# lukifer23/Matrix0

Hardware: AMD Instinct MI355X
Metric: self-play games/sec at 800 sims/move, ResNet-24 53M; 1/2/4/8 MI355X (higher is better)
Workload: dtype f16

## Files before the change

### matrix0_amd/csrc/capi_selfplay.hip

```cpp
#include <string.h>
#include <algorithm>
#include <memory>
#include "selfplay_engine.h"

using namespace m0;

static void fill_tree_cfg(const m0_selfplay_cfg& c, bool match, TreeCfg& t) {
    t.fpu_reduction = c.fpu_reduction; t.draw_penalty = c.draw_penalty; t.virtual_loss = c.virtual_loss;
    t.selection_jitter = c.selection_jitter; t.cpuct = c.cpuct; t.cpuct_start = c.cpuct_start; t.cpuct_end = c.cpuct_end;
    t.cpuct_plies = c.cpuct_plies; t.use_c_base = c.use_c_base; t.cpuct_c_base = c.cpuct_c_base; t.cpuct_c_init = c.cpuct_c_init;
    t.dirichlet_alpha = c.dirichlet_alpha; t.dirichlet_frac = c.dirichlet_frac; t.legal_softmax = c.legal_softmax;
    t.enable_entropy_noise = c.enable_entropy_noise; t.no_instant_backtrack = c.no_instant_backtrack;
    t.virtual_loss_active = c.virtual_loss_active; t.leaves_per_step = c.inference_batch_size;
    t.tt_merge = c.tt_merge; t.raw_legal_priors = c.raw_legal_priors; t.max_children = c.max_children;
    t.min_child_prior = c.min_child_prior;
    t.eval_cache = ((match ? c.arena_eval_cache : c.eval_cache) && c.legal_softmax && !c.raw_legal_priors && !c.tt_merge) ? 1 : 0;
}

static void alloc_tree_arenas(m0_selfplay* sp) {
    const m0_selfplay_cfg& c = sp->cfg;
    long want = c.arena_nodes > 0 ? c.arena_nodes : (long)(c.num_simulations * 1.3 + 64) * 96;
    if (want < 4096) want = 4096;
    sp->cap = (int)want;
    const size_t N = (size_t)sp->G * 2 * sp->cap;
    TreeArrays& t = sp->d.t;
    t.cap = sp->cap;
    t.prior = dalloc<double>(sp, N); t.w = dalloc<double>(sp, N); t.q = dalloc<double>(sp, N);
    t.n = dalloc<int>(sp, N); t.vl = dalloc<int>(sp, N); t.cbase = dalloc<int>(sp, N);
    t.nch = dalloc<int16_t>(sp, N); t.mv = dalloc<uint16_t>(sp, N); t.midx = dalloc<uint16_t>(sp, N);
    sp->d.games = dalloc<GameDev>(sp, sp->G);
    const size_t LS = (size_t)sp->L + 1;
    sp->d.samples = dalloc<Sample>(sp, (size_t)sp->G * LS);
    sp->d.paths = dalloc<int>(sp, (size_t)sp->G * LS * M0_MAX_DEPTH);
    sp->d.leaf_moves = dalloc<uint16_t>(sp, (size_t)sp->G * LS * M0_MAX_CHILDREN);
}

static bool alloc_position_tables(m0_selfplay* sp) {
    sp->d.tt_sides = 1;
    if (!sp->cfg.tt_merge) return true;
    const size_t LS = (size_t)sp->L + 1;
    int tc = 1024;
    while (tc < 2 * sp->cap) tc <<= 1;
    sp->d.tt_cap = tc;
    sp->d.tt_sides = sp->kind == EngineKind::Match ? 2 : 1;
    sp->d.search_nodes = (int)std::min<long>((long)sp->cfg.num_simulations * 48 + 4 * M0_MAX_CHILDREN, (long)sp->cap / 2);
    sp->d.epaths = dalloc<int>(sp, (size_t)sp->G * LS * M0_MAX_DEPTH);
    sp->d.tt_keys = dalloc<uint64_t>(sp, (size_t)sp->G * sp->d.tt_sides * tc);
    sp->d.tt_nodes = dalloc<int>(sp, (size_t)sp->G * sp->d.tt_sides * tc);
    if (sp->d.epaths && sp->d.tt_keys && sp->d.tt_nodes) return true;
    m0_set_error("hipMalloc failed for the position tables (tt_merge): lower concurrent_games or arena_nodes");
    return false;
}

static bool alloc_eval_cache(m0_selfplay* sp) {
    if (!sp->tc.eval_cache) return true;
    const size_t LS = (size_t)sp->L + 1;
    int entries = sp->cfg.eval_cache_entries > 0 ? sp->cfg.eval_cache_entries : 16384;
    int sets = 64;
    while (sets * 4 < entries) sets <<= 1;
    EvalCache& ec = sp->d.ec;
    ec.sets = sets;
    ec.sides = sp->kind == EngineKind::Match ? 2 : 1;
    const size_t entries_all = (size_t)sp->G * ec.sides * sets * 4;
    ec.keys = dalloc<uint64_t>(sp, entries_all);
    ec.stamps = dalloc<uint32_t>(sp, entries_all);
    ec.payload = dalloc<float>(sp, entries_all * M0_EC_WORDS);
    ec.hit_stage = dalloc<float>(sp, (size_t)sp->G * LS * M0_EC_WORDS);
    if (ec.keys && ec.stamps && ec.payload && ec.hit_stage) return true;
    m0_set_error("hipMalloc failed for the evaluation cache: lower eval_cache_entries or concurrent_games");
    return false;
}

static bool alloc_batch_buffers(m0_selfplay* sp) {
    const int nreg = sp->kind == EngineKind::Match ? 2 : 1;
    sp->d.hist = dalloc<uint64_t>(sp, (size_t)sp->G * M0_HIST_CAP);
    sp->d.results = dalloc<RootResult>(sp, sp->G);
    sp->d.row_counter = dalloc<int>(sp, 4);
    sp->d.x0 = dalloc<_Float16>(sp, (size_t)(nreg * sp->rows_max + 4) * 64 * 32);
    sp->logits_dev = dalloc<float>(sp, (size_t)nreg * sp->rows_max * 4672);
    sp->values_dev = dalloc<float>(sp, (size_t)nreg * sp->rows_max + 4);
    sp->d.net_row_base = sp->rows_max;
    if (sp->cfg.ssl_in_forward && sp->net && sp->net->ssl_channels_total() > 0)
        sp->ssl_dev = dalloc<float>(sp, (size_t)sp->rows_max * sp->net->ssl_channels_total() * 64);
    if (sp->cfg.ssl_targets) {
        sp->ssl_cap = sp->cfg.max_game_len > 0 ? sp->cfg.max_game_len + 1 : 513;
        sp->ssl_pos_dev = dalloc<Pos>(sp, sp->ssl_cap);
        sp->ssl_out_dev = dalloc<float>(sp, (size_t)sp->ssl_cap * 17 * 64);
        if (!sp->ssl_pos_dev || !sp->ssl_out_dev) {
            m0_set_error("hipMalloc failed for the SSL target staging buffers");
            return false;
        }
    }
    sp->ids_dev = dalloc<int>(sp, sp->G);
    sp->roots_dev = dalloc<int>(sp, sp->G);
    sp->d.logits = sp->logits_dev; sp->d.values = sp->values_dev;
    sp->d.G = sp->G; sp->d.L = sp->L;
    return true;
}

static bool make_tail_view(m0_selfplay* sp) {
    if (!(sp->cfg.tail_split && sp->net && sp->kind != EngineKind::Match && sp->net->cfg().channels > 256 && sp->net->cfg().channels <= 320 &&
          sp->rows_max >= 2048)) return true;
    if (create_stream_cu_mask_env("M0_TAIL_CU_MASK", &sp->stream_tail) != hipSuccess ||
        hipEventCreateWithFlags(&sp->ev_sel, hipEventDisableTiming) != hipSuccess ||
        hipEventCreateWithFlags(&sp->ev_tail, hipEventDisableTiming) != hipSuccess) {
        m0_set_error("hipStreamCreate / hipEventCreate failed (tail split)");
        return false;
    }
    sp->net_tail = sp->net->shared_view(sp->stream_tail);
    std::string werr;
    sp->half_split = sp->cfg.tail_split == 2;
    if (sp->net_tail->ensure_workspace(sp->half_split ? sp->rows_max / 2 + 1024 : 1023, werr) != M0_OK) {
        m0_set_error("tail split: " + werr);
        return false;
    }
    return true;
}
// ... 318 lines not shown
```

### matrix0_amd/csrc/tree.h

```cpp
#pragma once
#include <hip/hip_runtime.h>
#include <stdint.h>
#include "chess_core.h"
namespace m0 { struct TbSet; }
#include "../../include/m0_engine.h"

#define M0_MAX_DEPTH 256
#define M0_HIST_CAP 192
#define M0_MAX_CHILDREN 256
constexpr int M0_NHWC_C = 32;

struct TreeCfg {
    double fpu_reduction;
    double draw_penalty;
    double virtual_loss;
    double selection_jitter;
    double cpuct;
    double cpuct_start, cpuct_end;
    int cpuct_plies;
    int use_c_base;
    double cpuct_c_base, cpuct_c_init;
    double dirichlet_alpha, dirichlet_frac;
    int legal_softmax;
    int enable_entropy_noise;
// ... 17 lines not shown
    int sets;
    int sides;
};

struct GameDev {
    m0::Pos root_pos;
    int root;
    int next;
    int arena;
    int active;
    int sims_done, sims_target;
    int need_dirichlet;
    int root_q_from_v;
    int flip_root_v;
    int root_fresh;
    int hist_len;
    int nsamples;
    int overflow;
    int finished;
    int root_n;
    double root_q;
    double root_v;
    uint64_t seed_jitter, seed_noise, seed_dir;
    uint64_t ctr_jitter, ctr_noise, ctr_dir;
    uint64_t evals;
    int net_id;
    int reinfer;
    uint64_t cache_hits;
    uint32_t cache_clock[2];
    int ec_clear;
    int side_next[2];
    int root_found;
    uint64_t tb_leaves;
};

enum SampleKind : int {
    SK_NONE = 0,
    SK_EVAL = 1,
    SK_ROOT_INIT = 2,
    SK_TERMINAL = 3,
    SK_ROOT_VALUE = 4,
    SK_CACHED = 5,
    SK_SHARED = 6,
};
M0_HD bool sample_owns_row(int kind) { return kind == SK_EVAL || kind == SK_ROOT_INIT || kind == SK_ROOT_VALUE; }
M0_HD bool sample_holds_inflight(int kind) { return kind == SK_EVAL || kind == SK_TERMINAL || kind == SK_CACHED || kind == SK_SHARED; }

struct Sample {
    m0::Pos pos;
    int kind;
    uint64_t ckey;
    int leaf;
    int depth;
    int row;
    int nlegal;
};
static_assert(sizeof(Sample) == 104, "the host copies Sample arrays device-to-host: the layout must not move");

struct TreeArrays {
    double* prior;
    double* w;
    double* q;
    int* n;
    int* vl;
    int* cbase;
    int16_t* nch;
    uint16_t* mv;
    uint16_t* midx;
    int cap;
};

struct RootResult {
    int nchild;
    int root_n;
    double root_q;
    int child_node[M0_MAX_CHILDREN];
    int child_n[M0_MAX_CHILDREN];
    uint16_t child_mv[M0_MAX_CHILDREN];
    uint16_t child_idx[M0_MAX_CHILDREN];
    double child_prior[M0_MAX_CHILDREN];
    double child_q[M0_MAX_CHILDREN];
};

struct TreeDev {
    TreeArrays t;
    GameDev* games;
    Sample* samples;
    int* paths;
    int* epaths;
    uint64_t* tt_keys;
    int* tt_nodes;
    int tt_cap;
    EvalCache ec;
    int search_nodes;
    int tt_sides;
    uint16_t* leaf_moves;
    uint64_t* hist;
    RootResult* results;
    int* row_counter;
    int net_row_base;
    _Float16* x0;
    const float* logits;
    const float* values;
    int G;
    int L;
    const m0::TbSet* tb_set;
    int tb_max_pieces;
};

hipError_t launch_select(const TreeDev& d, const TreeCfg& c, hipStream_t st);
hipError_t launch_expand(const TreeDev& d, const TreeCfg& c, hipStream_t st);
enum RootMode : int {
    ROOT_FRESH = -1,
    ROOT_FROM_SIDE_TABLE = -2,
    ROOT_FIRST_OF_GAME = -3,
};
hipError_t launch_advance(const TreeDev& d, const int* game_ids_dev, const int* child_slots_dev, int count, hipStream_t st);

hipError_t launch_encode_positions(const m0::Pos* pos_dev, int n, float* planes_f32_dev ,
                                   _Float16* nhwc_dev , uint8_t* mask_dev ,
                                   int32_t* nlegal_dev, uint16_t* moves_dev , int32_t* idx_dev ,
                                   hipStream_t st);

hipError_t launch_decode_planes(const float* planes_dev, const uint8_t* mask_dev, int n, m0::Pos* pos_dev, int32_t* status_dev,
                                int32_t* flags_dev, int32_t* nlegal_dev, hipStream_t st);

hipError_t launch_analysis_lines(const TreeDev& d, const int* slots_dev, int count, int multipv, int pv_len,
                                 m0_analysis_line* lines_dev, int* nlines_dev, hipStream_t st);
hipError_t launch_root_children(const TreeDev& d, const int* slots_dev, int count, int32_t* policy_idx_dev, int32_t* visits_dev,
                                int32_t* nchild_dev, hipStream_t st);
hipError_t launch_policy_lines(const float* logits_dev, const float* values_dev, const int32_t* nlegal_dev, const uint16_t* moves_dev,
                               const int32_t* idx_dev, int rows, int multipv, m0_analysis_line* lines_dev, int* nlines_dev,
                               float* value_out_dev, hipStream_t st);

hipError_t launch_ssl_targets(const m0::Pos* pos_dev, int n, float* out_dev, hipStream_t st);

hipError_t launch_replay_games(const m0::Pos* start_dev, const uint32_t* patterns_dev, const int32_t* offsets_dev ,
                               int n_games, int max_plies, m0::Pos* pos_dev, uint16_t* moves_dev, int32_t* policy_idx_dev,
                               int32_t* nlegal_dev, int8_t* turn_dev, int32_t* plies_dev, int32_t* status_dev,
                               int32_t* end_flags_dev, hipStream_t st);
```

### matrix0_amd/csrc/tree_device.h

```cpp
#pragma once
#include <hip/hip_runtime.h>
#include <math.h>
#include "tree.h"

using namespace m0;

#define GOLDEN64 0x9E3779B97F4A7C15ull

__device__ __forceinline__ double u01(uint64_t seed, uint64_t k) {
    return (double)(mix64(seed + (k + 1) * GOLDEN64) >> 11) * (1.0 / 9007199254740992.0);
}
__device__ __forceinline__ double normal_at(uint64_t seed, uint64_t k) {
    double u1 = u01(seed, k), u2 = u01(seed, k + 1);
    if (u1 < 1e-300) u1 = 1e-300;
    return sqrt(-2.0 * log(u1)) * cos(2.0 * 3.141592653589793 * u2);
}
static __device__ double gamma_draw(uint64_t seed, uint64_t& ctr, double a) {
    double boost = 1.0;
    if (a < 1.0) {
        double u = u01(seed, ctr++);
        boost = pow(u, 1.0 / a);
        a += 1.0;
    }
    const double d = a - 1.0 / 3.0, c = 1.0 / sqrt(9.0 * d);
    for (int it = 0; it < 1000; ++it) {
        double x = normal_at(seed, ctr); ctr += 2;
        double v = 1.0 + c * x;
        if (v <= 0.0) continue;
        v = v * v * v;
        double u = u01(seed, ctr++);
        if (u < 1e-300) u = 1e-300;
        if (log(u) < 0.5 * x * x + d - d * v + d * log(v)) return d * v * boost;
    }
    return d * boost;
}

struct Arena {
    double* prior; double* w; double* q; int* n; int* vl; int* cbase; int16_t* nch; uint16_t* mv; uint16_t* midx;
};
__device__ __forceinline__ Arena arena_of(const TreeArrays& t, int g, int half) {
    size_t b = ((size_t)g * 2 + half) * (size_t)t.cap;
    Arena a;
    a.prior = t.prior + b; a.w = t.w + b; a.q = t.q + b; a.n = t.n + b; a.vl = t.vl + b;
    a.cbase = t.cbase + b; a.nch = t.nch + b; a.mv = t.mv + b; a.midx = t.midx + b;
    return a;
}
__device__ __forceinline__ void node_reset(const Arena& A, int i, double prior, Move mv, uint16_t midx) {
    A.prior[i] = prior; A.w[i] = 0.0; A.q[i] = 0.0; A.n[i] = 0; A.vl[i] = 0;
    A.cbase[i] = -1; A.nch[i] = -1; A.mv[i] = mv; A.midx[i] = midx;
}
__device__ __forceinline__ void node_copy(const Arena& D, int dn, const Arena& S, int so) {
    D.prior[dn] = S.prior[so]; D.w[dn] = S.w[so]; D.q[dn] = S.q[so]; D.n[dn] = S.n[so]; D.vl[dn] = 0;
    D.cbase[dn] = S.cbase[so]; D.nch[dn] = S.nch[so]; D.mv[dn] = S.mv[so]; D.midx[dn] = S.midx[so];
}

__device__ __forceinline__ float wave_max_f(float v) {
    for (int o = 32; o > 0; o >>= 1) v = fmaxf(v, __shfl_xor(v, o));
    return v;
}
__device__ __forceinline__ float wave_sum_f(float v) {
    for (int o = 32; o > 0; o >>= 1) v += __shfl_xor(v, o);
    return v;
}
__device__ __forceinline__ double wave_sum_d(double v) {
    for (int o = 32; o > 0; o >>= 1) v += __shfl_xor(v, o);
    return v;
}

constexpr int CPL = M0_MAX_CHILDREN / 64;
static_assert(M0_POLICY_SIZE % 4 == 0, "logit rows are read as 16-byte pieces");

__device__ __forceinline__ bool row_nonfinite(const float* lg, int lane) {
    constexpr int N4 = M0_POLICY_SIZE / 4, PER_LANE = (N4 + 63) / 64;
    const uint4* lg4 = reinterpret_cast<const uint4*>(lg);
    uint4 v[PER_LANE];
#pragma unroll
    for (int k = 0; k < PER_LANE; ++k) { const int j = lane + 64 * k; v[k] = lg4[j < N4 ? j : N4 - 1]; }
    uint32_t acc = 0;
#pragma unroll
    for (int k = 0; k < PER_LANE; ++k) {
        acc |= (uint32_t)((v[k].x & 0x7f800000u) == 0x7f800000u) | (uint32_t)((v[k].y & 0x7f800000u) == 0x7f800000u) |
               (uint32_t)((v[k].z & 0x7f800000u) == 0x7f800000u) | (uint32_t)((v[k].w & 0x7f800000u) == 0x7f800000u);
    }
    return acc != 0;
}

__device__ __forceinline__ void wave_softmax(const float (&l)[CPL], int n, int lane, float (&pr)[CPL]) {
    float mx = -3.0e38f;
#pragma unroll
    for (int k = 0; k < CPL; ++k) mx = fmaxf(mx, l[k]);
    mx = wave_max_f(mx);
    double e[CPL], sum = 0.0;
#pragma unroll
    for (int k = 0; k < CPL; ++k) { const int i = lane + 64 * k; e[k] = i < n ? exp((double)(l[k] - mx)) : 0.0; sum += e[k]; }
    sum = wave_sum_d(sum);
#pragma unroll
    for (int k = 0; k < CPL; ++k) pr[k] = (float)(e[k] / sum);
}

__device__ __forceinline__ int reserve_row(const TreeDev& d, const GameDev* gd, int lane) {
    int row = 0;
    if (lane == 0) row = atomicAdd(d.row_counter + gd->net_id, 1) + gd->net_id * d.net_row_base;
    return __shfl(row, 0);
}
__device__ __forceinline__ double root_value(const GameDev* gd, float v) {
    double rv = fmax(-1.0, fmin(1.0, (double)v));
    if (gd->flip_root_v) rv = -rv;
    return rv;
}

__device__ __forceinline__ uint64_t tt_key_of(const Pos& p) { const uint64_t k = tkey(p); return k ? k : 1ull; }
__device__ __forceinline__ int tt_home(uint64_t key, int cap) { return (int)((key ^ (key >> 29)) & (uint64_t)(cap - 1)); }
__device__ __forceinline__ size_t tt_table_of(const TreeDev& d, int g, const GameDev* gd) {
    return ((size_t)g * d.tt_sides + (d.tt_sides == 2 ? gd->arena : 0)) * (size_t)d.tt_cap;
}
__device__ __forceinline__ void tt_clear(uint64_t* keys, int nkeys, int lane) {
    uint4* tk = reinterpret_cast<uint4*>(keys);
    for (int i = lane; i < nkeys / 2; i += 64) tk[i] = make_uint4(0, 0, 0, 0);
}
static __device__ int tt_lookup(const uint64_t* keys, const int* nodes, int cap, uint64_t key, int lane) {
    const int mask = cap - 1, home = tt_home(key, cap);
    for (int it = 0; it < cap; it += 64) {
        const uint64_t k = keys[(home + it + lane) & mask];
        const unsigned long long hit = __ballot(k == key), emp = __ballot(k == 0ull);
        const int fh = hit ? __builtin_ctzll(hit) : 64, fe = emp ? __builtin_ctzll(emp) : 64;
        if (fh < fe) return nodes[(home + it + fh) & mask];
        if (fe < 64) return -1;
    }
    return -1;
}
static __device__ void tt_insert(uint64_t* keys, int* nodes, int cap, uint64_t key, int node) {
    const int mask = cap - 1;
    int s = tt_home(key, cap);
    for (int it = 0; it < cap; ++it) {
        const unsigned long long prev = atomicCAS(reinterpret_cast<unsigned long long*>(keys + s), 0ull, (unsigned long long)key);
        if (prev == 0ull || prev == (unsigned long long)key) { nodes[s] = node; return; }
        s = (s + 1) & mask;
    }
}

struct NoMirror { __device__ __forceinline__ void operator()(int, int, double) const {} };
template <typename Mirror>
static __device__ void backprop(const Arena& A, const int* path, int depth, double value, int lane, bool may_repeat,
                                const Mirror& mirror) {
    const double v = fmax(-1.0, fmin(1.0, value));
    if (may_repeat) {
        bool dup = false;
        for (int d = lane; d <= depth; d += 64) {
            const int nd = path[d];
// ... 26 lines not shown
```

### matrix0_amd/csrc/tree_expand.hip

```cpp
#include "tree_device.h"
#include "eval_cache.h"

struct ExpandScratch {
    float pr[M0_MAX_CHILDREN];
    uint8_t keep[M0_MAX_CHILDREN];
    float total;
    int bad;
};

struct ExpandEnv {
    Arena A;
    int cap;
    GameDev* gd;
    uint64_t* TK; int* TN; int tt_cap;
    ExpandScratch* X;
    int lane;
};
struct LeafLogits {
    const float* row;
    const float* legal;
    float* store;
};
__device__ __forceinline__ LeafLogits logits_of_row(const float* row, float* store) { return LeafLogits{row, nullptr, store}; }
__device__ __forceinline__ LeafLogits logits_of_cache(const float* payload) { return LeafLogits{nullptr, payload + EC_LOGITS, nullptr}; }

static __device__ float np_sum_f32_dev(const float* a, int n) {
    auto block = [&](const float* b, int m) -> float {
        if (m < 8) { float r = 0.f; for (int i = 0; i < m; ++i) r += b[i]; return r; }
        float r[8];
        for (int j = 0; j < 8; ++j) r[j] = b[j];
        int i;
        for (i = 8; i < m - (m % 8); i += 8)
            for (int j = 0; j < 8; ++j) r[j] += b[i + j];
        float res = ((r[0] + r[1]) + (r[2] + r[3])) + ((r[4] + r[5]) + (r[6] + r[7]));
        for (; i < m; ++i) res += b[i];
        return res;
    };
    if (n <= 128) return block(a, n);
    int n2 = n / 2;
    n2 -= n2 % 8;
    return block(a, n2) + block(a + n2, n - n2);
}

__device__ __forceinline__ void priors_raw(const float* lg, const int (&idx)[CPL], int n, int lane, ExpandScratch* X, float (&pr)[CPL]) {
#pragma unroll
    for (int k = 0; k < CPL; ++k) { const int i = lane + 64 * k; if (i < n) X->pr[i] = lg[idx[k]]; }
    __syncthreads();
    if (lane == 0) X->total = np_sum_f32_dev(X->pr, n);
    __syncthreads();
    const float total = X->total;
    const bool ok = isfinite(total) && total > 0.f;
#pragma unroll
    for (int k = 0; k < CPL; ++k) { const int i = lane + 64 * k; pr[k] = i < n ? (ok ? X->pr[i] / total : 1.0f / (float)n) : 0.f; }
    __syncthreads();
}

__device__ __forceinline__ void priors_uniform(int n, float (&pr)[CPL]) {
#pragma unroll
    for (int k = 0; k < CPL; ++k) pr[k] = 1.0f / (float)n;
}

__device__ __forceinline__ void priors_legal_softmax(const LeafLogits& src, const int (&idx)[CPL], int n, int lane, GameDev* gd,
                                                     const TreeCfg& c, float (&pr)[CPL]) {
    double ent = 0.0;
    float l[CPL];
#pragma unroll
    for (int k = 0; k < CPL; ++k) {
        const int i = lane + 64 * k;
        l[k] = i < n ? (src.legal ? src.legal[i] : src.row[idx[k]]) : -3.0e38f;
        if (src.store && i < n && i < M0_EC_MAXLEGAL) src.store[EC_LOGITS + i] = l[k];
    }
    wave_softmax(l, n, lane, pr);
#pragma unroll
    for (int k = 0; k < CPL; ++k) {
        const int i = lane + 64 * k;
        if (i < n) ent -= (double)pr[k] * log((double)pr[k] + 1e-8);
    }
    ent = wave_sum_d(ent);
    const double ratio = ent / fmax(1e-9, log((double)(n > 1 ? n : 1)));
    if (c.enable_entropy_noise && ratio > 0.9) {
        const uint64_t ctr = gd->ctr_noise;
        const uint64_t seed = gd->seed_noise;
        double dd[CPL], ds = 0.0;
#pragma unroll
        for (int k = 0; k < CPL; ++k) {
            const int i = lane + 64 * k;
            dd[k] = 0.0;
            if (i < n) { dd[k] = fmax((double)pr[k] + 0.1 * normal_at(seed, ctr + 2ull * (uint64_t)i), 1e-8); ds += dd[k]; }
        }
        ds = wave_sum_d(ds);
#pragma unroll
        for (int k = 0; k < CPL; ++k) pr[k] = (float)(dd[k] / ds);
        if (lane == 0) gd->ctr_noise = ctr + 2ull * (uint64_t)n;
    }
}

__device__ __forceinline__ void priors_full_softmax(const float* lg, const int (&idx)[CPL], int n, int lane, GameDev* gd,
                                                    const TreeCfg& c, float (&pr)[CPL]) {
    float mx = -3.0e38f;
    double ent = 0.0;
    for (int j = lane; j < M0_POLICY_SIZE; j += 64) mx = fmaxf(mx, lg[j]);
    mx = wave_max_f(mx);
    double sum = 0.0;
    for (int j = lane; j < M0_POLICY_SIZE; j += 64) sum += exp((double)(lg[j] - mx));
    sum = wave_sum_d(sum);
    const double fsum = sum;
    for (int j = lane; j < M0_POLICY_SIZE; j += 64) {
        const double pj = (double)(float)(exp((double)(lg[j] - mx)) / sum);
        ent -= pj * log(pj + 1e-8);
    }
#pragma unroll
    for (int k = 0; k < CPL; ++k) { const int i = lane + 64 * k; pr[k] = i < n ? (float)(exp((double)(lg[idx[k]] - mx)) / sum) : 0.f; }
    ent = wave_sum_d(ent);
    const double ratio = ent / fmax(1e-9, log((double)(n > 1 ? n : 1)));
    if (c.enable_entropy_noise && ratio > 0.9) {
        const uint64_t ctr = gd->ctr_noise;
        const uint64_t seed = gd->seed_noise;
        double ds = 0.0;
        for (int j = lane; j < M0_POLICY_SIZE; j += 64)
            ds += fmax((double)(float)(exp((double)(lg[j] - mx)) / fsum) + 0.1 * normal_at(seed, ctr + 2ull * (uint64_t)j), 1e-8);
        ds = wave_sum_d(ds);
#pragma unroll
        for (int k = 0; k < CPL; ++k) {
            const int i = lane + 64 * k;
            if (i < n) {
                const int j = idx[k];
                pr[k] = (float)(fmax((double)pr[k] + 0.1 * normal_at(seed, ctr + 2ull * (uint64_t)j), 1e-8) / ds);
            }
        }
        if (lane == 0) gd->ctr_noise = ctr + 2ull * (uint64_t)M0_POLICY_SIZE;
    }
}

__device__ __forceinline__ void priors_renormalise(int n, int lane, float (&pr)[CPL]) {
    double tot = 0.0;
#pragma unroll
    for (int k = 0; k < CPL; ++k) { const int i = lane + 64 * k; if (i < n) { if (!(pr[k] >= 0.f) || !isfinite(pr[k])) pr[k] = 0.f; tot += (double)pr[k]; } }
    tot = wave_sum_d(tot);
    const float totf = (float)tot;
    if (totf > 0.f && isfinite(totf)) {
#pragma unroll
        for (int k = 0; k < CPL; ++k) pr[k] = pr[k] / totf;
    } else priors_uniform(n, pr);
}

__device__ __forceinline__ int prune_children(const TreeCfg& c, const float (&pr)[CPL], int n, int lane, ExpandScratch* X, int (&slot)[CPL]) {
#pragma unroll
    for (int k = 0; k < CPL; ++k) slot[k] = lane + 64 * k;
    if (!(c.max_children > 0 || c.min_child_prior > 0.0)) return n;
#pragma unroll
    for (int k = 0; k < CPL; ++k) {
        const int i = lane + 64 * k;
        if (i < n) { X->pr[i] = pr[k]; X->keep[i] = (c.min_child_prior > 0.0 && !((double)pr[k] >= c.min_child_prior)) ? 0 : 1; }
    }
    __syncthreads();
    int kept = 0;
    for (int j = 0; j < n; ++j) kept += X->keep[j];
    const bool topk = c.max_children > 0 && kept > c.max_children;
    const int nkeep = topk ? c.max_children : kept;
#pragma unroll
    for (int k = 0; k < CPL; ++k) {
        const int i = lane + 64 * k;
        slot[k] = -1;
        if (i < n && X->keep[i]) {
            int r = 0;
            if (topk) { for (int j = 0; j < n; ++j) r += (X->keep[j] && (X->pr[j] > pr[k] || (X->pr[j] == pr[k] && j < i))) ? 1 : 0; }
            else { for (int j = 0; j < i; ++j) r += X->keep[j]; }
            if (r < nkeep) slot[k] = r;
        }
    }
    __syncthreads();
    return nkeep;
}

__device__ __forceinline__ bool write_children(const ExpandEnv& E, int leaf, const Pos& pos, const Move (&mvv)[CPL], const int (&idx)[CPL],
                                               const float (&pr)[CPL], const int (&slot)[CPL], int n, int nkeep, bool reg_children) {
    const Arena& A = E.A;
    GameDev* gd = E.gd;
    const int lane = E.lane;
    const int cb = gd->next;
    if (cb + nkeep > E.cap) { if (lane == 0) gd->overflow = 1; return false; }
#pragma unroll
    for (int k = 0; k < CPL; ++k) {
        const int i = lane + 64 * k;
        if (i < n && slot[k] >= 0) {
            const int ci = cb + slot[k];
            node_reset(A, ci, (double)pr[k], mvv[k], (uint16_t)idx[k]);
            if (E.TK && reg_children) {
                Pos q = pos;
                make_move(q, mvv[k]);
                tt_insert(E.TK, E.TN, E.tt_cap, tt_key_of(q), ci);
            }
        }
    }
    if (E.TK && !reg_children && lane == 0) tt_insert(E.TK, E.TN, E.tt_cap, tt_key_of(pos), leaf);
    if (lane == 0) { A.cbase[leaf] = cb; A.nch[leaf] = (int16_t)nkeep; gd->next = cb + nkeep; }
    __syncthreads();
    return true;
}

__device__ __forceinline__ bool expand_node(const ExpandEnv& E, const TreeCfg& c, int leaf, const Pos& pos, const uint16_t* smoves, int n,
                                   const LeafLogits& src, bool is_root, bool reg_children) {
    const int lane = E.lane;
    if (n <= 0) return true;
    bool bad = false;
    if (!src.legal) bad = row_nonfinite(src.row, lane);
    bad = __any(bad);
    if (lane == 0) E.X->bad = bad ? 1 : 0;
    float pr[CPL];
    int idx[CPL];
    Move mvv[CPL];
#pragma unroll
    for (int k = 0; k < CPL; ++k) {
        const int i = lane + 64 * k;
        pr[k] = 0.f; idx[k] = 0; mvv[k] = 0;
        if (i < n) { mvv[k] = smoves[i]; idx[k] = move_to_index(pos, mvv[k]); }
    }
    if (c.raw_legal_priors && c.legal_softmax && !is_root) priors_raw(src.row, idx, n, lane, E.X, pr);
    else if (bad) priors_uniform(n, pr);
    else {
        if (c.legal_softmax) priors_legal_softmax(src, idx, n, lane, E.gd, c, pr);
        else priors_full_softmax(src.row, idx, n, lane, E.gd, c, pr);
        priors_renormalise(n, lane, pr);
    }
    int slot[CPL];
    const int nkeep = prune_children(c, pr, n, lane, E.X, slot);
    return write_children(E, leaf, pos, mvv, idx, pr, slot, n, nkeep, reg_children);
}

__device__ __forceinline__ void expand_evaluated(const TreeDev& d, const TreeCfg& c, const ExpandEnv& E, int g, const Sample& smp,
                                                 const uint16_t* moves, const float* lg, float v) {
    const Arena& A = E.A;
    GameDev* gd = E.gd;
    const int lane = E.lane, kind = smp.kind, leaf = smp.leaf;
    const Pos pos = smp.pos;
    float* cw = nullptr;
    size_t ce = 0;
    const uint64_t ckey = kind == SK_EVAL ? smp.ckey : 0ull;
    if (ckey != 0 && isfinite(v)) {
        ce = ec_choose_victim(d.ec, gd, g, ckey, lane);
        cw = ec_payload(d.ec, ce);
        ec_invalidate(d.ec, ce, lane);
    }
    const bool ok = expand_node(E, c, leaf, pos, moves, smp.nlegal, logits_of_row(lg, cw), kind == SK_ROOT_INIT,
                                !(kind == SK_ROOT_INIT && gd->root_fresh));
    if (c.eval_cache && kind == SK_EVAL && lane == 0 && A.nch[leaf] < 0) A.cbase[leaf] = -1;
    const int sig = cw ? legal_sig(moves, smp.nlegal, lane) : 0;
    if (cw && lane == 0) {
        if (ok && !E.X->bad) ec_publish(d.ec, gd, ce, ckey, v, sig);
    }
}

__device__ __forceinline__ void release_inflight(const TreeDev& d, const TreeCfg& c, const Arena& A, int g, const Sample* S, const int* P,
                                                 int ns, int lane) {
    for (int s = lane; s < ns; s += 64) {
        if (sample_holds_inflight(S[s].kind)) {
            const int* path = (c.tt_merge ? d.epaths + (size_t)g * (d.L + 1) * M0_MAX_DEPTH : P) + (size_t)s * M0_MAX_DEPTH;
            for (int dd = 1; dd <= S[s].depth; ++dd) atomicSub(&A.vl[path[dd]], 1);
        }
    }
}

__device__ __forceinline__ void write_root_result(RootResult* R, const Arena& A, int root, int lane) {
    const int k = A.nch[root] > 0 ? A.nch[root] : 0;
    const int cb = A.cbase[root];
    for (int i = lane; i < k; i += 64) {
        R->child_node[i] = cb + i; R->child_n[i] = A.n[cb + i];
        R->child_mv[i] = A.mv[cb + i]; R->child_idx[i] = A.midx[cb + i];
        R->child_prior[i] = A.prior[cb + i]; R->child_q[i] = A.q[cb + i];
    }
    if (lane == 0) { R->nchild = k; R->root_n = A.n[root]; R->root_q = A.q[root]; }
}

__global__ __launch_bounds__(64) void expand_kernel(TreeDev d, TreeCfg c) {
    __shared__ ExpandScratch X;
    const int g = blockIdx.x, lane = threadIdx.x;
    GameDev* gd = &d.games[g];
    if (!gd->active) return;
    uint64_t* TK = c.tt_merge ? d.tt_keys + tt_table_of(d, g, gd) : nullptr;
    int* TN = c.tt_merge ? d.tt_nodes + tt_table_of(d, g, gd) : nullptr;
    const uint16_t* LM = d.leaf_moves + (size_t)g * (d.L + 1) * M0_MAX_CHILDREN;
    const int ns = gd->nsamples;
    if (ns <= 0) return;
    const Arena A = arena_of(d.t, g, gd->arena);
    const ExpandEnv E{A, d.t.cap, gd, TK, TN, d.tt_cap, &X, lane};
    const Sample* S = d.samples + (size_t)g * (d.L + 1);
    const int* P = d.paths + (size_t)g * (d.L + 1) * M0_MAX_DEPTH;
    const bool may_repeat = c.tt_merge != 0;
    int sims = 0;
    uint64_t evals = 0, hits = 0;
    for (int s = 0; s < ns; ++s) {
        const int kind = S[s].kind;
        const int* path = P + (size_t)s * M0_MAX_DEPTH;
        const uint16_t* moves = LM + (size_t)s * M0_MAX_CHILDREN;
        if (kind == SK_SHARED) {
            const float v = d.values[S[s].row];
            backprop(A, path, S[s].depth, (double)v, lane, may_repeat, NoMirror{});
            ++sims; ++hits;
            __syncthreads();
        } else if (kind == SK_CACHED) {
            const int leaf = S[s].leaf, depth = S[s].depth;
            const float* pay = ec_hit_stage(d, g, s);
            const float v = pay[EC_VALUE];
            if (A.nch[leaf] < 0) {
                const Pos pos = S[s].pos;
                expand_node(E, c, leaf, pos, moves, S[s].nlegal, logits_of_cache(pay), false, true);
            }
            backprop(A, path, depth, (double)v, lane, may_repeat, NoMirror{});
            ++sims; ++hits;
            __syncthreads();
        } else if (kind == SK_EVAL || kind == SK_ROOT_INIT) {
            const int leaf = S[s].leaf, depth = S[s].depth, row = S[s].row;
            const float* lg = d.logits + (size_t)row * M0_POLICY_SIZE;
            const float v = d.values[row];
            if (A.nch[leaf] < 0) expand_evaluated(d, c, E, g, S[s], moves, lg, v);
            ++evals;
            if (kind == SK_EVAL) {
                backprop(A, path, depth, (double)v, lane, may_repeat, NoMirror{});
                ++sims;
            } else {
                const double rv = root_value(gd, v);
                if (lane == 0) {
                    gd->root_v = rv;
                    if (gd->root_q_from_v) { A.q[leaf] = rv; gd->root_q_from_v = 0; }
                }
            }
            __syncthreads();
        } else if (kind == SK_TERMINAL) {
            ++sims;
        } else if (kind == SK_ROOT_VALUE) {
            const double rv = root_value(gd, d.values[S[s].row]);
            if (lane == 0) gd->root_v = rv;
            ++evals;
        }
    }
    if (c.virtual_loss_active) release_inflight(d, c, A, g, S, P, ns, lane);
    __syncthreads();
    const int done = gd->sims_done + sims;
    const int root = gd->root;
    const bool fin = (A.nch[root] >= 0 || gd->overflow) && done >= gd->sims_target;
    if (lane == 0) {
        gd->sims_done = done;
        gd->evals += evals;
        gd->cache_hits += hits;
        gd->finished = fin ? 1 : 0;
        gd->root_n = A.n[root];
        gd->root_q = A.q[root];
    }
    if (fin) write_root_result(d.results + g, A, root, lane);
}

hipError_t launch_expand(const TreeDev& d, const TreeCfg& c, hipStream_t st) {
    hipLaunchKernelGGL(expand_kernel, dim3(d.G), dim3(64), 0, st, d, c);
    return hipGetLastError();
}
```

### matrix0_amd/csrc/tree_select.hip

```cpp
#include "tree_device.h"
#include "tb_core.h"
#include "eval_cache.h"
#include "movegen_wave.h"
#include "kernel_common.h"

__device__ __forceinline__ double cpuct_at(const TreeCfg& c, int ply) {
    if (c.use_c_base) {
        double N = fmax(1.0, (double)(ply + 1));
        return c.cpuct_c_init + log((N + c.cpuct_c_base) / c.cpuct_c_base);
    }
    if (c.cpuct_plies <= 0) return c.cpuct;
    int p = ply < 0 ? 0 : (ply > c.cpuct_plies ? c.cpuct_plies : ply);
    double t = (double)p / (double)c.cpuct_plies;
    return c.cpuct_start + (c.cpuct_end - c.cpuct_start) * t;
}
static __device__ void apply_dirichlet(const Arena& A, int root, GameDev* gd, const TreeCfg& c, double* sg, int lane) {
    const int k = A.nch[root];
    if (k <= 0 || c.dirichlet_frac <= 0.0) return;
    const int cb = A.cbase[root];
    uint64_t ctr = gd->ctr_dir;
    double sum = 0.0;
    for (int i = 0; i < k; ++i) {
        double gmm = gamma_draw(gd->seed_dir, ctr, c.dirichlet_alpha);
        if (lane == 0) sg[i] = gmm;
// ... 114 lines not shown

__global__ __launch_bounds__(64) void select_kernel(TreeDev d, TreeCfg c) {
    extern __shared__ __attribute__((aligned(16))) char sel_cache[];
    TopCache* const TC = reinterpret_cast<TopCache*>(sel_cache);
    __shared__ uint64_t pkey[M0_MAX_DEPTH];
    __shared__ uint8_t pirr[M0_MAX_DEPTH];
    __shared__ Move smoves[M0_MAX_MOVES];
    __shared__ Move spseudo[M0_MAX_MOVES];
    __shared__ double sg[M0_MAX_CHILDREN];
    const int g = blockIdx.x, lane = threadIdx.x;
    GameDev* gd = &d.games[g];
    if (!gd->active) { if (lane == 0) gd->nsamples = 0; return; }
    uint16_t* LM = d.leaf_moves + (size_t)g * (d.L + 1) * M0_MAX_CHILDREN;
    const Arena A = arena_of(d.t, g, gd->arena);
    const int root = gd->root;
    Sample* S = d.samples + (size_t)g * (d.L + 1);
    int* P = d.paths + (size_t)g * (d.L + 1) * M0_MAX_DEPTH;
    int* EP = c.tt_merge ? d.epaths + (size_t)g * (d.L + 1) * M0_MAX_DEPTH : nullptr;
    const uint64_t* TK = c.tt_merge ? d.tt_keys + tt_table_of(d, g, gd) : nullptr;
    const int* TN = c.tt_merge ? d.tt_nodes + tt_table_of(d, g, gd) : nullptr;
    const bool reinfer = gd->reinfer != 0;

    if (A.nch[root] < 0) { emit_root_init(d, gd, S, P, LM, root, reinfer, smoves, spseudo, lane); return; }
    if (gd->need_dirichlet) {
        apply_dirichlet(A, root, gd, c, sg, lane);
        if (lane == 0) gd->need_dirichlet = 0;
    }
    int nleaf = gd->sims_target - gd->sims_done;
    if (nleaf > d.L) nleaf = d.L;
    if (nleaf < 0) nleaf = 0;
    int ncached = 0;
    if (!c.tt_merge && nleaf > 0) {
        ncached = gd->next < M0_SEL_CACHE ? gd->next : M0_SEL_CACHE;
        for (int i = lane; i < ncached; i += 64) {
            TC->prior[i] = A.prior[i]; TC->q[i] = A.q[i]; TC->n[i] = A.n[i]; TC->vl[i] = A.vl[i]; TC->cbase[i] = A.cbase[i];
            TC->nch[i] = A.nch[i]; TC->mv[i] = A.mv[i];
        }
        __syncthreads();
    }
    uint64_t ctrj = gd->ctr_jitter;
    const uint64_t seedj = gd->seed_jitter;
    const double jit = c.selection_jitter > 0.0 ? c.selection_jitter : 0.001;
    const int hist_len = gd->hist_len;
    const uint64_t* H = d.hist + (size_t)g * M0_HIST_CAP;

    for (int s = 0; s < nleaf; ++s) {
        Pos pos = gd->root_pos;
        int* path = P + (size_t)s * M0_MAX_DEPTH;
        int* epath = c.tt_merge ? EP + (size_t)s * M0_MAX_DEPTH : nullptr;
        int node = root, depth = 0;
        int prev_from = -1, prev_to = -1;
        if (lane == 0) { path[0] = root; if (epath) epath[0] = root; }
        const bool rh = node < ncached;
        int nc = TOP(nch, rh, node), cb = TOP(cbase, rh, node), nn = TOP(n, rh, node);
        double nq = TOP(q, rh, node);
        while (true) {
            if (nc <= 0 || depth >= M0_MAX_DEPTH - 1) break;
            const double sq = sqrt((double)(nn > 1 ? nn : 1));
            const double eff = cpuct_at(c, depth);
            double best = -1e9;
            int bi = -1;
            int b_nch = 0, b_cb = 0, b_n = 0, b_vl = 0;
            double b_q = 0.0;
            Move b_mv = 0;
            for (int i = lane; i < nc; i += 64) {
                const int ci = cb + i;
                const bool hit = ci < ncached;
                const int cn = TOP(n, hit, ci);
                const double cq = TOP(q, hit, ci);
                const int c_nch = TOP(nch, hit, ci), c_cb = TOP(cbase, hit, ci);
                const Move m = TOP(mv, hit, ci);
                const double cprior = TOP(prior, hit, ci);
                const double qq = cn == 0 ? nq - c.fpu_reduction : cq;
                const double u = eff * cprior * (sq / (1.0 + (double)cn));
                double sc = qq + u;
                if (c.no_instant_backtrack && depth >= 1) {
                    if (mv_from(m) == prev_to && mv_to(m) == prev_from) sc -= 0.01;
                }
                const int cvl = c.virtual_loss_active ? TOP(vl, hit, ci) : 0;
                if (c.virtual_loss_active && c.virtual_loss > 0.0) sc -= (double)cvl * c.virtual_loss;
                sc += (u01(seedj, ctrj + (uint64_t)i) - 0.5) * jit;
                if (sc > best) { best = sc; bi = i; b_nch = c_nch; b_cb = c_cb; b_n = cn; b_q = cq; b_mv = m; b_vl = cvl; }
            }
            for (int off = 32; off > 0; off >>= 1) {
                const double ob = __shfl_xor(best, off);
                const int oi = __shfl_xor(bi, off);
                if (oi >= 0 && (bi < 0 || ob > best || (ob == best && oi < bi))) { best = ob; bi = oi; }
            }
            ctrj += (uint64_t)nc;
            if (bi < 0) bi = 0;
            const int child = cb + bi;
            const int wl = bi & 63;
            nc = __shfl(b_nch, wl); cb = __shfl(b_cb, wl); nn = __shfl(b_n, wl); nq = __shfl(b_q, wl);
            const Move m = (Move)__shfl((int)b_mv, wl);
            const uint64_t k = tkey(pos);
            const bool irr = irreversible(pos, m);
            if (lane == 0) { pkey[depth] = k; pirr[depth] = irr ? 1 : 0; }
            make_move(pos, m);
            const int vlw = __shfl(b_vl, wl);
            if (lane == 0 && c.virtual_loss_active) { A.vl[child] = vlw + 1; if (child < ncached) TC->vl[child] = vlw + 1; }
            prev_from = mv_from(m); prev_to = mv_to(m);
            node = child; ++depth;
            if (c.tt_merge) {
                const int tn = tt_lookup(TK, TN, d.tt_cap, tt_key_of(pos), lane);
                if (tn >= 0 && tn != child) {
                    node = tn;
                    nc = A.nch[node]; cb = A.cbase[node]; nn = A.n[node]; nq = A.q[node];
                }
                if (lane == 0) epath[depth] = child;
            }
            if (lane == 0) path[depth] = node;
        }
        __syncthreads();
        const int nlegal = gen_legal_wave(pos, smoves, spseudo, lane);
        double tv;
        bool tb_hit;
        const bool term = leaf_terminal(d, c, pos, nlegal, depth, pkey, pirr, H, hist_len, lane, tv, tb_hit);
        if (tb_hit && lane == 0) gd->tb_leaves++;
        uint64_t ckey = 0;
        bool cached = false;
        if (!term && c.eval_cache && d.ec.sets > 0 && nlegal <= M0_EC_MAXLEGAL) {
            ckey = ec_key_of(pos);
            cached = ec_probe(d, gd, g, s, ckey, smoves, nlegal, lane);
        }
        emit_leaf(d, c, A, gd, S + s, LM + (size_t)s * M0_MAX_CHILDREN, pos, node, depth, smoves, nlegal, term, cached, ckey, lane);
        __syncthreads();
        if (term) {
            backprop(A, path, depth, tv, lane, c.tt_merge != 0, [&](int nd, int nn, double qq) {
                if (nd < ncached) { TC->n[nd] = nn; TC->q[nd] = qq; }
            });
            __syncthreads();
            __builtin_amdgcn_fence(__ATOMIC_ACQUIRE, "agent");
        }
    }
    if (reinfer) emit_root_value(d, gd, S, nleaf, root, lane);
    if (lane == 0) { gd->ctr_jitter = ctrj; gd->nsamples = nleaf + (reinfer ? 1 : 0); }
}

hipError_t launch_select(const TreeDev& d, const TreeCfg& c, hipStream_t st) {
    static DeviceOnce once;
    hipError_t e = once.run([] {
        return hipFuncSetAttribute(reinterpret_cast<const void*>(&select_kernel), hipFuncAttributeMaxDynamicSharedMemorySize, M0_SEL_CACHE_BYTES);
    });
    if (e != hipSuccess) return e;
    hipLaunchKernelGGL(select_kernel, dim3(d.G), dim3(64), M0_SEL_CACHE_BYTES, st, d, c);
    return hipGetLastError();
}
```

Measured before the change: 1.142.

## Precompute leaf priors in parallel kernels and use DPP wave argmax in select

Adds two pre-pass kernels that run one wavefront per (game, sample) to compute legal-softmax priors, non-finite checks, move indices and entropy noise. The per-game expand kernel then consumes these instead of doing the work serially across samples. The noise counter offset is derived from a prefix sum so results match the serial order. Separately, select replaces the shfl-based argmax and broadcast with DPP row ops and readlane. This adds extra launches, a per-sample buffer and a fallback path when the precomputed counter no longer matches.

```diff
diff --git a/matrix0_amd/csrc/argmax_order.h b/matrix0_amd/csrc/argmax_order.h
--- /dev/null
+++ b/matrix0_amd/csrc/argmax_order.h
@@ -0,0 +1,10 @@
+#pragma once
+#if defined(__HIPCC__)
+#define M0_ARGMAX_HD __host__ __device__ inline
+#else
+#define M0_ARGMAX_HD inline
+#endif
+
+M0_ARGMAX_HD bool argmax_beats(double ob, int oi, double best, int bi) {
+    return oi >= 0 && (bi < 0 || ob > best || (ob == best && oi < bi));
+}
diff --git a/matrix0_amd/csrc/capi_selfplay.hip b/matrix0_amd/csrc/capi_selfplay.hip
--- a/matrix0_amd/csrc/capi_selfplay.hip
+++ b/matrix0_amd/csrc/capi_selfplay.hip
@@ -33,6 +33,9 @@
     sp->d.samples = dalloc<Sample>(sp, (size_t)sp->G * LS);
     sp->d.paths = dalloc<int>(sp, (size_t)sp->G * LS * M0_MAX_DEPTH);
     sp->d.leaf_moves = dalloc<uint16_t>(sp, (size_t)sp->G * LS * M0_MAX_CHILDREN);
+    const char* split = getenv("M0_EXPAND_SPLIT");
+    if (!(split && split[0] == '0') && sp->tc.legal_softmax && !sp->tc.raw_legal_priors && !sp->tc.tt_merge)
+        sp->d.lp = dalloc<LeafPriors>(sp, (size_t)sp->G * LS);
 }
 
 static bool alloc_position_tables(m0_selfplay* sp) {
diff --git a/matrix0_amd/csrc/tree.h b/matrix0_amd/csrc/tree.h
--- a/matrix0_amd/csrc/tree.h
+++ b/matrix0_amd/csrc/tree.h
@@ -123,8 +123,20 @@
     double child_q[M0_MAX_CHILDREN];
 };
 
+struct LeafPriors {
+    float pr[M0_MAX_CHILDREN];
+    float lg[M0_MAX_CHILDREN];
+    uint16_t idx[M0_MAX_CHILDREN];
+    uint64_t ctr_base;
+    int cand;
+    int bad;
+    int fires;
+    int valid;
+};
+
 struct TreeDev {
     TreeArrays t;
+    LeafPriors* lp;
     GameDev* games;
     Sample* samples;
     int* paths;
diff --git a/matrix0_amd/csrc/tree_device.h b/matrix0_amd/csrc/tree_device.h
--- a/matrix0_amd/csrc/tree_device.h
+++ b/matrix0_amd/csrc/tree_device.h
@@ -2,6 +2,7 @@
 #include <hip/hip_runtime.h>
 #include <math.h>
 #include "tree.h"
+#include "argmax_order.h"
 
 using namespace m0;
 
@@ -62,9 +63,45 @@
     for (int o = 32; o > 0; o >>= 1) v += __shfl_xor(v, o);
     return v;
 }
+__device__ __forceinline__ int wave_sum_i(int v) {
+    for (int o = 32; o > 0; o >>= 1) v += __shfl_xor(v, o);
+    return v;
+}
 __device__ __forceinline__ double wave_sum_d(double v) {
     for (int o = 32; o > 0; o >>= 1) v += __shfl_xor(v, o);
     return v;
+}
+
+template <int CTRL>
+__device__ __forceinline__ int dpp_i(int v) { return __builtin_amdgcn_update_dpp(0, v, CTRL, 0xF, 0xF, true); }
+__device__ __forceinline__ int readlane_i(int v, int l) { return __builtin_amdgcn_readlane(v, l); }
+__device__ __forceinline__ double readlane_d(double v, int l) {
+    const uint64_t u = __builtin_bit_cast(uint64_t, v);
+    const uint32_t lo = (uint32_t)readlane_i((int)(uint32_t)u, l), hi = (uint32_t)readlane_i((int)(uint32_t)(u >> 32), l);
+    return __builtin_bit_cast(double, (uint64_t)hi << 32 | lo);
+}
+template <int CTRL>
+__device__ __forceinline__ void argmax_dpp_step(double& best, int& bi) {
+    const uint64_t u = __builtin_bit_cast(uint64_t, best);
+    const uint32_t lo = (uint32_t)dpp_i<CTRL>((int)(uint32_t)u), hi = (uint32_t)dpp_i<CTRL>((int)(uint32_t)(u >> 32));
+    const double ob = __builtin_bit_cast(double, (uint64_t)hi << 32 | lo);
+    const int oi = dpp_i<CTRL>(bi);
+    if (argmax_beats(ob, oi, best, bi)) { best = ob; bi = oi; }
+}
+__device__ __forceinline__ void wave_argmax(double& best, int& bi) {
+    argmax_dpp_step<0xB1>(best, bi);
+    argmax_dpp_step<0x4E>(best, bi);
+    argmax_dpp_step<0x141>(best, bi);
+    argmax_dpp_step<0x140>(best, bi);
+    double rb = readlane_d(best, 0);
+    int ri = readlane_i(bi, 0);
+#pragma unroll
+    for (int row = 1; row < 4; ++row) {
+        const double ob = readlane_d(best, 16 * row);
+        const int oi = readlane_i(bi, 16 * row);
+        if (argmax_beats(ob, oi, rb, ri)) { rb = ob; ri = oi; }
+    }
+    best = rb; bi = ri;
 }
 
 constexpr int CPL = M0_MAX_CHILDREN / 64;
diff --git a/matrix0_amd/csrc/tree_expand.hip b/matrix0_amd/csrc/tree_expand.hip
--- a/matrix0_amd/csrc/tree_expand.hip
+++ b/matrix0_amd/csrc/tree_expand.hip
@@ -60,37 +60,44 @@
     for (int k = 0; k < CPL; ++k) pr[k] = 1.0f / (float)n;
 }
 
+__device__ __forceinline__ bool legal_softmax_flat(const LeafLogits& src, const int (&idx)[CPL], int n, int lane, float (&l)[CPL],
+                                                   float (&pr)[CPL]) {
+    double ent = 0.0;
+#pragma unroll
+    for (int k = 0; k < CPL; ++k) {
+        const int i = lane + 64 * k;
+        l[k] = i < n ? (src.legal ? src.legal[i] : src.row[idx[k]]) : -3.0e38f;
+        if (src.store && i < n && i < M0_EC_MAXLEGAL) src.store[EC_LOGITS + i] = l[k];
+    }
+    wave_softmax(l, n, lane, pr);
+#pragma unroll
+    for (int k = 0; k < CPL; ++k) {
+        const int i = lane + 64 * k;
+        if (i < n) ent -= (double)pr[k] * log((double)pr[k] + 1e-8);
+    }
+    ent = wave_sum_d(ent);
+    const double ratio = ent / fmax(1e-9, log((double)(n > 1 ? n : 1)));
+    return ratio > 0.9;
+}
+__device__ __forceinline__ void entropy_noise(int n, int lane, uint64_t seed, uint64_t ctr, float (&pr)[CPL]) {
+    double dd[CPL], ds = 0.0;
+#pragma unroll
+    for (int k = 0; k < CPL; ++k) {
+        const int i = lane + 64 * k;
+        dd[k] = 0.0;
+        if (i < n) { dd[k] = fmax((double)pr[k] + 0.1 * normal_at(seed, ctr + 2ull * (uint64_t)i), 1e-8); ds += dd[k]; }
+    }
+    ds = wave_sum_d(ds);
+#pragma unroll
+    for (int k = 0; k < CPL; ++k) pr[k] = (float)(dd[k] / ds);
+}
 __device__ __forceinline__ void priors_legal_softmax(const LeafLogits& src, const int (&idx)[CPL], int n, int lane, GameDev* gd,
                                                      const TreeCfg& c, float (&pr)[CPL]) {
-    double ent = 0.0;
     float l[CPL];
-#pragma unroll
-    for (int k = 0; k < CPL; ++k) {
-        const int i = lane + 64 * k;
-        l[k] = i < n ? (src.legal ? src.legal[i] : src.row[idx[k]]) : -3.0e38f;
-        if (src.store && i < n && i < M0_EC_MAXLEGAL) src.store[EC_LOGITS + i] = l[k];
-    }
-    wave_softmax(l, n, lane, pr);
-#pragma unroll
-    for (int k = 0; k < CPL; ++k) {
-        const int i = lane + 64 * k;
-        if (i < n) ent -= (double)pr[k] * log((double)pr[k] + 1e-8);
-    }
-    ent = wave_sum_d(ent);
-    const double ratio = ent / fmax(1e-9, log((double)(n > 1 ? n : 1)));
-    if (c.enable_entropy_noise && ratio > 0.9) {
+    const bool flat = legal_softmax_flat(src, idx, n, lane, l, pr);
+    if (c.enable_entropy_noise && flat) {
         const uint64_t ctr = gd->ctr_noise;
-        const uint64_t seed = gd->seed_noise;
-        double dd[CPL], ds = 0.0;
-#pragma unroll
-        for (int k = 0; k < CPL; ++k) {
-            const int i = lane + 64 * k;
-            dd[k] = 0.0;
-            if (i < n) { dd[k] = fmax((double)pr[k] + 0.1 * normal_at(seed, ctr + 2ull * (uint64_t)i), 1e-8); ds += dd[k]; }
-        }
-        ds = wave_sum_d(ds);
-#pragma unroll
-        for (int k = 0; k < CPL; ++k) pr[k] = (float)(dd[k] / ds);
+        entropy_noise(n, lane, gd->seed_noise, ctr, pr);
         if (lane == 0) gd->ctr_noise = ctr + 2ull * (uint64_t)n;
     }
 }
@@ -199,29 +206,64 @@
     return true;
 }
 
+__device__ __forceinline__ bool logits_nonfinite(const LeafLogits& src, int lane) {
+    bool bad = false;
+    if (!src.legal) bad = row_nonfinite(src.row, lane);
+    return __any(bad);
+}
+__device__ __forceinline__ void leaf_move_indices(const Pos& pos, const uint16_t* smoves, int n, int lane, Move (&mvv)[CPL], int (&idx)[CPL]) {
+#pragma unroll
+    for (int k = 0; k < CPL; ++k) {
+        const int i = lane + 64 * k;
+        idx[k] = 0; mvv[k] = 0;
+        if (i < n) { mvv[k] = smoves[i]; idx[k] = move_to_index(pos, mvv[k]); }
+    }
+}
+
+__device__ __forceinline__ bool precomputed_holds(const LeafPriors* pre, const GameDev* gd) {
+    if (!pre || !pre->valid) return false;
+    const bool ok = !pre->fires || pre->ctr_base == __hip_atomic_load(&gd->ctr_noise, __ATOMIC_RELAXED, __HIP_MEMORY_SCOPE_AGENT);
+    return __builtin_amdgcn_readfirstlane((int)ok) != 0;
+}
+__device__ __forceinline__ void take_precomputed(const ExpandEnv& E, const LeafPriors& pre, const uint16_t* smoves, int n, float* store,
+                                                 Move (&mvv)[CPL], int (&idx)[CPL], float (&pr)[CPL]) {
+    const int lane = E.lane;
+#pragma unroll
+    for (int k = 0; k < CPL; ++k) {
+        const int i = lane + 64 * k;
+        pr[k] = 0.f; idx[k] = 0; mvv[k] = 0;
+        if (i < n) {
+            mvv[k] = smoves[i]; idx[k] = pre.idx[i]; pr[k] = pre.pr[i];
+            if (store && !pre.bad && i < M0_EC_MAXLEGAL) store[EC_LOGITS + i] = pre.lg[i];
+        }
+    }
+    if (lane == 0) {
+        E.X->bad = pre.bad;
+        if (pre.fires) E.gd->ctr_noise = pre.ctr_base + 2ull * (uint64_t)n;
+    }
+}
+
 __device__ __forceinline__ bool expand_node(const ExpandEnv& E, const TreeCfg& c, int leaf, const Pos& pos, const uint16_t* smoves, int n,
-                                   const LeafLogits& src, bool is_root, bool reg_children) {
+                                   const LeafLogits& src, bool is_root, bool reg_children, const LeafPriors* pre) {
     const int lane = E.lane;
     if (n <= 0) return true;
-    bool bad = false;
-    if (!src.legal) bad = row_nonfinite(src.row, lane);
-    bad = __any(bad);
-    if (lane == 0) E.X->bad = bad ? 1 : 0;
     float pr[CPL];
     int idx[CPL];
     Move mvv[CPL];
-#pragma unroll
-    for (int k = 0; k < CPL; ++k) {
-        const int i = lane + 64 * k;
-        pr[k] = 0.f; idx[k] = 0; mvv[k] = 0;
-        if (i < n) { mvv[k] = smoves[i]; idx[k] = move_to_index(pos, mvv[k]); }
-    }
-    if (c.raw_legal_priors && c.legal_softmax && !is_root) priors_raw(src.row, idx, n, lane, E.X, pr);
-    else if (bad) priors_uniform(n, pr);
+    if (precomputed_holds(pre, E.gd)) take_precomputed(E, *pre, smoves, n, src.store, mvv, idx, pr);
     else {
-        if (c.legal_softmax) priors_legal_softmax(src, idx, n, lane, E.gd, c, pr);
-        else priors_full_softmax(src.row, idx, n, lane, E.gd, c, pr);
-        priors_renormalise(n, lane, pr);
+        const bool bad = logits_nonfinite(src, lane);
+        if (lane == 0) E.X->bad = bad ? 1 : 0;
+#pragma unroll
+        for (int k = 0; k < CPL; ++k) pr[k] = 0.f;
+        leaf_move_indices(pos, smoves, n, lane, mvv, idx);
+        if (c.raw_legal_priors && c.legal_softmax && !is_root) priors_raw(src.row, idx, n, lane, E.X, pr);
+        else if (bad) priors_uniform(n, pr);
+        else {
+            if (c.legal_softmax) priors_legal_softmax(src, idx, n, lane, E.gd, c, pr);
+            else priors_full_softmax(src.row, idx, n, lane, E.gd, c, pr);
+            priors_renormalise(n, lane, pr);
+        }
     }
     int slot[CPL];
     const int nkeep = prune_children(c, pr, n, lane, E.X, slot);
@@ -229,7 +271,7 @@
 }
 
 __device__ __forceinline__ void expand_evaluated(const TreeDev& d, const TreeCfg& c, const ExpandEnv& E, int g, const Sample& smp,
-                                                 const uint16_t* moves, const float* lg, float v) {
+                                                 const uint16_t* moves, const float* lg, float v, const LeafPriors* pre) {
     const Arena& A = E.A;
     GameDev* gd = E.gd;
     const int lane = E.lane, kind = smp.kind, leaf = smp.leaf;
@@ -243,7 +285,7 @@
         ec_invalidate(d.ec, ce, lane);
     }
     const bool ok = expand_node(E, c, leaf, pos, moves, smp.nlegal, logits_of_row(lg, cw), kind == SK_ROOT_INIT,
-                                !(kind == SK_ROOT_INIT && gd->root_fresh));
+                                !(kind == SK_ROOT_INIT && gd->root_fresh), pre);
     if (c.eval_cache && kind == SK_EVAL && lane == 0 && A.nch[leaf] < 0) A.cbase[leaf] = -1;
     const int sig = cw ? legal_sig(moves, smp.nlegal, lane) : 0;
     if (cw && lane == 0) {
@@ -270,6 +312,74 @@
         R->child_prior[i] = A.prior[cb + i]; R->child_q[i] = A.q[cb + i];
     }
     if (lane == 0) { R->nchild = k; R->root_n = A.n[root]; R->root_q = A.q[root]; }
+}
+
+__device__ __forceinline__ bool sample_expands(int kind) { return kind == SK_EVAL || kind == SK_ROOT_INIT || kind == SK_CACHED; }
+
+__global__ __launch_bounds__(64) void expand_priors_kernel(TreeDev d, TreeCfg c) {
+    const int LS = d.L + 1, g = blockIdx.x / LS, s = blockIdx.x % LS, lane = threadIdx.x;
+    const GameDev* gd = &d.games[g];
+    if (!gd->active || s >= gd->nsamples) return;
+    const Sample* S = d.samples + (size_t)g * LS;
+    LeafPriors* lp = d.lp + (size_t)g * LS + s;
+    const int kind = S[s].kind, leaf = S[s].leaf, n = S[s].nlegal;
+    const Arena A = arena_of(d.t, g, gd->arena);
+    bool cand = sample_expands(kind) && n > 0 && A.nch[leaf] < 0;
+    if (cand) {
+        bool dup = false;
+        for (int e = lane; e < s; e += 64) dup = dup || (S[e].leaf == leaf && sample_expands(S[e].kind));
+        cand = !__any(dup);
+    }
+    if (lane == 0) { lp->cand = cand ? 1 : 0; lp->valid = 0; }
+    if (!cand) return;
+    const Pos pos = S[s].pos;
+    const uint16_t* moves = d.leaf_moves + ((size_t)g * LS + s) * M0_MAX_CHILDREN;
+    const LeafLogits src = kind == SK_CACHED ? logits_of_cache(ec_hit_stage(d, g, s))
+                                             : logits_of_row(d.logits + (size_t)S[s].row * M0_POLICY_SIZE, nullptr);
+    const bool bad = logits_nonfinite(src, lane);
+    int idx[CPL];
+    Move mvv[CPL];
+    leaf_move_indices(pos, moves, n, lane, mvv, idx);
+    float l[CPL], pr[CPL];
+    bool flat = false;
+    if (!bad) flat = legal_softmax_flat(src, idx, n, lane, l, pr);
+#pragma unroll
+    for (int k = 0; k < CPL; ++k) {
+        const int i = lane + 64 * k;
+        if (i < n) {
+            lp->idx[i] = (uint16_t)idx[k];
+            if (!bad) { lp->pr[i] = pr[k]; lp->lg[i] = l[k]; }
+        }
+    }
+    if (lane == 0) { lp->bad = bad ? 1 : 0; lp->fires = (!bad && c.enable_entropy_noise && flat) ? 1 : 0; }
+}
+
+__global__ __launch_bounds__(64) void expand_noise_kernel(TreeDev d, TreeCfg c) {
+    const int LS = d.L + 1, g = blockIdx.x / LS, s = blockIdx.x % LS, lane = threadIdx.x;
+    const GameDev* gd = &d.games[g];
+    if (!gd->active || s >= gd->nsamples) return;
+    const Sample* S = d.samples + (size_t)g * LS;
+    LeafPriors* L0 = d.lp + (size_t)g * LS;
+    LeafPriors* lp = L0 + s;
+    if (!lp->cand) return;
+    const int n = S[s].nlegal;
+    float pr[CPL];
+    if (lp->bad) priors_uniform(n, pr);
+    else {
+#pragma unroll
+        for (int k = 0; k < CPL; ++k) { const int i = lane + 64 * k; pr[k] = i < n ? lp->pr[i] : 0.f; }
+        if (lp->fires) {
+            int adv = 0;
+            for (int e = lane; e < s; e += 64) if (L0[e].cand && L0[e].fires) adv += 2 * S[e].nlegal;
+            const uint64_t ctr = gd->ctr_noise + (uint64_t)wave_sum_i(adv);
+            entropy_noise(n, lane, gd->seed_noise, ctr, pr);
+            if (lane == 0) lp->ctr_base = ctr;
+        }
+        priors_renormalise(n, lane, pr);
+    }
+#pragma unroll
+    for (int k = 0; k < CPL; ++k) { const int i = lane + 64 * k; if (i < n) lp->pr[i] = pr[k]; }
+    if (lane == 0) lp->valid = 1;
 }
 
 __global__ __launch_bounds__(64) void expand_kernel(TreeDev d, TreeCfg c) {
@@ -293,6 +403,7 @@
         const int kind = S[s].kind;
         const int* path = P + (size_t)s * M0_MAX_DEPTH;
         const uint16_t* moves = LM + (size_t)s * M0_MAX_CHILDREN;
+        const LeafPriors* pre = d.lp ? d.lp + (size_t)g * (d.L + 1) + s : nullptr;
         if (kind == SK_SHARED) {
             const float v = d.values[S[s].row];
             backprop(A, path, S[s].depth, (double)v, lane, may_repeat, NoMirror{});
@@ -304,7 +415,7 @@
             const float v = pay[EC_VALUE];
             if (A.nch[leaf] < 0) {
                 const Pos pos = S[s].pos;
-                expand_node(E, c, leaf, pos, moves, S[s].nlegal, logits_of_cache(pay), false, true);
+                expand_node(E, c, leaf, pos, moves, S[s].nlegal, logits_of_cache(pay), false, true, pre);
             }
             backprop(A, path, depth, (double)v, lane, may_repeat, NoMirror{});
             ++sims; ++hits;
@@ -313,7 +424,7 @@
             const int leaf = S[s].leaf, depth = S[s].depth, row = S[s].row;
             const float* lg = d.logits + (size_t)row * M0_POLICY_SIZE;
             const float v = d.values[row];
-            if (A.nch[leaf] < 0) expand_evaluated(d, c, E, g, S[s], moves, lg, v);
+            if (A.nch[leaf] < 0) expand_evaluated(d, c, E, g, S[s], moves, lg, v, pre);
             ++evals;
             if (kind == SK_EVAL) {
                 backprop(A, path, depth, (double)v, lane, may_repeat, NoMirror{});
@@ -351,6 +462,10 @@
 }
 
 hipError_t launch_expand(const TreeDev& d, const TreeCfg& c, hipStream_t st) {
+    if (d.lp) {
+        hipLaunchKernelGGL(expand_priors_kernel, dim3(d.G * (d.L + 1)), dim3(64), 0, st, d, c);
+        hipLaunchKernelGGL(expand_noise_kernel, dim3(d.G * (d.L + 1)), dim3(64), 0, st, d, c);
+    }
     hipLaunchKernelGGL(expand_kernel, dim3(d.G), dim3(64), 0, st, d, c);
     return hipGetLastError();
 }
diff --git a/matrix0_amd/csrc/tree_select.hip b/matrix0_amd/csrc/tree_select.hip
--- a/matrix0_amd/csrc/tree_select.hip
+++ b/matrix0_amd/csrc/tree_select.hip
@@ -220,22 +220,18 @@
                 sc += (u01(seedj, ctrj + (uint64_t)i) - 0.5) * jit;
                 if (sc > best) { best = sc; bi = i; b_nch = c_nch; b_cb = c_cb; b_n = cn; b_q = cq; b_mv = m; b_vl = cvl; }
             }
-            for (int off = 32; off > 0; off >>= 1) {
-                const double ob = __shfl_xor(best, off);
-                const int oi = __shfl_xor(bi, off);
-                if (oi >= 0 && (bi < 0 || ob > best || (ob == best && oi < bi))) { best = ob; bi = oi; }
-            }
+            wave_argmax(best, bi);
             ctrj += (uint64_t)nc;
             if (bi < 0) bi = 0;
             const int child = cb + bi;
-            const int wl = bi & 63;
-            nc = __shfl(b_nch, wl); cb = __shfl(b_cb, wl); nn = __shfl(b_n, wl); nq = __shfl(b_q, wl);
-            const Move m = (Move)__shfl((int)b_mv, wl);
+            const int wl = __builtin_amdgcn_readfirstlane(bi & 63);
+            nc = readlane_i(b_nch, wl); cb = readlane_i(b_cb, wl); nn = readlane_i(b_n, wl); nq = readlane_d(b_q, wl);
+            const Move m = (Move)readlane_i((int)b_mv, wl);
             const uint64_t k = tkey(pos);
             const bool irr = irreversible(pos, m);
             if (lane == 0) { pkey[depth] = k; pirr[depth] = irr ? 1 : 0; }
             make_move(pos, m);
-            const int vlw = __shfl(b_vl, wl);
+            const int vlw = readlane_i(b_vl, wl);
             if (lane == 0 && c.virtual_loss_active) { A.vl[child] = vlw + 1; if (child < ncached) TC->vl[child] = vlw + 1; }
             prev_from = mv_from(m); prev_to = mv_to(m);
             node = child; ++depth;
```

Result: no change. 1.147, median of 6 (+0.4%).
